# Sidharthshanu/Gossip-protocol-with-power-law

Hardware: AMD Instinct MI355X
Metric: gossip edge-deliveries/s (GTEPS) & HBM roofline %, 2^24 nodes x 4096 msgs (higher is better)
Workload: dtype u64

## Files before the change

### gossip-protocol-with-power-law_amd/csrc/driver.hip

```cpp
#include <hip/hip_runtime.h>

#include <cstdlib>
#include <rccl/rccl.h>

#include <algorithm>
#include <cmath>
#include <cstring>
#include <string>
#include <vector>

#include "gp_device.h"
#include "xplan.h"

namespace gp {

static thread_local std::string g_err;
int set_error(int code, const std::string& msg) {
  g_err = msg;
  return code;
}
int copy_sync(Ctx* c, void* dst, const void* src, size_t bytes, hipMemcpyKind kind) {
  if (bytes == 0) return 0;
  GP_HIP(hipMemcpyAsync(dst, src, bytes, kind, c->stream));
  GP_HIP(hipStreamSynchronize(c->stream));
// ... 268 lines not shown
  a.lm_next = c->lm_write_now ? c->d_lmw[c->cur ^ 1] : nullptr;
  a.cmk = c->cml_read_now ? c->d_cmk[c->cur] : nullptr;
  a.cml = c->cml_read_now ? c->d_cml[c->cur] : nullptr;
  a.cmk_next = c->cml_write_now ? c->d_cmk[c->cur ^ 1] : nullptr;
  a.cml_next = c->cml_write_now ? c->d_cml[c->cur ^ 1] : nullptr;
  a.frx = c->d_frx[0] ? c->d_frx[c->cur] : nullptr;
  a.frx_next = c->d_frx[0] ? c->d_frx[c->cur ^ 1] : nullptr;
  a.frx_rows = c->frx_rows;
  a.done_at = c->d_done_at;
  a.gcol = c->d_gcol;
  a.midx = c->d_midx;
  a.cmask = c->d_cmask;
  a.early_exit = c->early_exit_now ? 1 : 0;
  a.dprobe = c->dprobe_now ? 1 : 0;
  a.alias = c->alias_now ? 1 : 0;
  a.ulist = c->ulist_read_now ? c->d_ulist[c->ul_cur] : nullptr;
  a.ulist_n = c->ulist_read_now ? c->ulist_n : 0;
  a.ulist_next = c->ulist_emit_now ? c->d_ulist[c->ul_cur ^ 1] : nullptr;
  a.fpop_next = c->d_fpop[c->cur ^ 1];
  a.seenpop = c->d_seenpop;
  a.first = c->cfg.track_first ? c->d_first : nullptr;
  a.digest = c->cfg.track_digest ? c->d_digest : nullptr;
  a.state = c->d_state;
  a.deg_live = c->d_deg_live;
  a.partial = c->d_stats + 64;
  a.hub_items = c->d_hub_items;
  a.hubs = c->d_hubs;
  a.hub_item_ptr = c->d_hub_item_ptr;
  a.hub_partial = c->d_hub_partial;
  a.hub_pnz = c->d_hub_pnz;
  a.hub_done = c->d_hub_done;
  if (++c->hub_epoch == 0) c->hub_epoch = 1;
  a.hub_epoch = c->hub_epoch;
  a.vbegin = 0;
  a.nloc = c->nloc();
  a.m_total = c->m;
  a.wbase = c->cfg.msg_word_base;
  a.rr = c->round + 1;
  a.hub_thr = c->cfg.hub_threshold;
  a.orp = c->directed ? c->d_out_row_ptr : c->d_row_ptr;
  a.ocol = c->directed ? c->d_out_col : c->d_col;
  a.acc = c->d_acc;
  a.tbits = c->d_tbits;
  a.touched = c->d_touched;
  a.active = c->d_active;
  a.big = c->d_big;
  a.stats = c->d_stats;
}


#ifndef GP_EE_DIV
#define GP_EE_DIV 16.0
#endif
#ifndef GP_EE_DIV_NARROW
#define GP_EE_DIV_NARROW 64.0
#endif
static int launch_expand(Ctx* c) {
  if (alive_on(c))
    GP_HIP(hipMemsetAsync(c->d_alive + (size_t)(c->cur ^ 1) * c->words, 0, (size_t)c->words * 8, c->stream));
  const int r = c->round;
  const double ee_div = c->words <= 8 ? GP_EE_DIV_NARROW : GP_EE_DIV;
  c->early_exit_now = c->cfg.early_exit != 0 &&
                      ((double)c->prev_new_bits * ee_div >= (double)c->n * (double)c->m ||
                       (double)c->held_bits * 2.0 >= (double)c->n * (double)c->m);
  const u64 inj = (size_t)r < c->inj_arcs.size() ? (u64)c->inj_arcs[(size_t)r] : 0ull;
  const double est = (double)((r == 0 ? 0ull : c->prev_next_arcs) + inj);
// ... 626 lines not shown
```

### gossip-protocol-with-power-law_amd/csrc/gp_device.h

```cpp
#pragma once
#include <hip/hip_runtime.h>

#include <algorithm>
#include <cstdint>

#include "gp_internal.h"

namespace gp {

typedef unsigned long long u64;
typedef u64 u64x2 __attribute__((ext_vector_type(2)));

constexpr int BLOCK = 256;
constexpr int WAVES = BLOCK / 64;
constexpr int GS = 256 / BLOCK;
#ifndef GP_EXPAND_BLOCK
#define GP_EXPAND_BLOCK 64
#endif
constexpr int EBLOCK = GP_EXPAND_BLOCK;
constexpr int EWAVES = EBLOCK / 64;
constexpr int HBLOCK = 256;
constexpr int HWAVES = HBLOCK / 64;
constexpr int NPART = 2048;

// ... 115 lines not shown
  const uint32_t* __restrict__ done_at;
  uint32_t* __restrict__ fpop_next;
  u64* __restrict__ frx;
  u64* __restrict__ frx_next;
  int64_t frx_rows;
  uint32_t* __restrict__ seenpop;
  uint8_t* __restrict__ first;
  u64* __restrict__ digest;
  uint8_t* __restrict__ state;
  const int32_t* __restrict__ deg_live;
  u64* __restrict__ partial;
  const HubItem* __restrict__ hub_items;
  const int32_t* __restrict__ hubs;
  const int32_t* __restrict__ hub_item_ptr;
  u64* __restrict__ hub_partial;
  uint32_t* __restrict__ hub_pnz;
  uint32_t* __restrict__ hub_done;
  uint32_t hub_epoch;
  const int64_t* __restrict__ orp;
  const int32_t* __restrict__ ocol;
  u64* __restrict__ acc;
  u64* __restrict__ tbits;
  const u64* __restrict__ nbits;
  int32_t* __restrict__ touched;
  const int32_t* __restrict__ active;
  const int32_t* __restrict__ big;
  u64* __restrict__ stats;
  int64_t vbegin, nloc;
  int64_t n_items;
  int32_t m_total;
  int32_t wbase;
  int32_t rr;
  int32_t hub_thr;
};

constexpr uint8_t SLOT_NONE = 0xFF;
constexpr uint8_t SLOT_PARKED = 2;
constexpr uint8_t SLOT_CMASK = 3;
constexpr uint8_t LMN_ALIAS = 0x10;

constexpr int CML_WORDS = 16;
constexpr int CML_MAXW = CML_WORDS - 1;

#ifndef GP_DETECT_BLOCKS_PER_CU
#define GP_DETECT_BLOCKS_PER_CU 16
#endif
constexpr double SUMMARY_RATIO = 256.0;
#define EXPAND_BOUNDS __launch_bounds__(EBLOCK)
#ifndef GP_ROWS_IN_FLIGHT
#define GP_ROWS_IN_FLIGHT 4
#endif
#ifndef GP_ROWS_IN_FLIGHT_64
#define GP_ROWS_IN_FLIGHT_64 3
#endif
#ifndef GP_ROWS_IN_FLIGHT_NARROW
#define GP_ROWS_IN_FLIGHT_NARROW 2
#endif
template <int W>
struct RowsInFlight {
  static constexpr int value = W >= 64 ? GP_ROWS_IN_FLIGHT_64 : W == 8 ? GP_ROWS_IN_FLIGHT_NARROW : GP_ROWS_IN_FLIGHT;
};

constexpr int PRE_IDS = 8;
constexpr int PRE_MAX_DEG = 16;
#ifndef GP_WAVE_PRE_MAX
#define GP_WAVE_PRE_MAX 64
// ... 519 lines not shown
    const uint32_t hi = (uint32_t)__shfl_xor((int)nib, 1);
    if (!(lane & 1) && li < a.nloc) a.lm_next[li >> 1] = (uint8_t)(nib | (hi << 4));
  }
  if constexpr (LDS::kCml) {
    if (a.cmk_next) {
      const u64 dm = __ballot(!need || L.tot[lane] == 0u || L.cd[lane] != 0);
      if (lane == 0 && li < a.nloc) a.cmk_next[li >> 6] = dm;
    }
  }
}



inline int grid_for(int64_t work, int64_t per_block) {
  int64_t g = (work + per_block - 1) / per_block;
  if (g < 1) g = 1;
  if (g > (int64_t)0x7fffffff) g = 0x7fffffff;
  return (int)g;
}
inline bool alive_on(const Ctx* c) { return c->d_alive != nullptr && c->liveness_active; }
inline bool alive_now(const Ctx* c) { return alive_on(c) && c->alive_from >= 0 && c->round >= c->alive_from; }
inline bool state_ready(const Ctx* c) { return c->d_sp != nullptr && c->d_slot[0] != nullptr; }

int launch_round_kernels(Ctx* c, const ExpandArgs& a);
template <int W> void launch_expand_flat_w(Ctx* c, const ExpandArgs& a);
void launch_expand_rec(Ctx* c, const ExpandArgs& a);
void launch_mklm(Ctx* c, const ExpandArgs& a);
void launch_arcmask(Ctx* c);
template <int W> void launch_fixup_rows_w(Ctx* c);
template <int W> void launch_park_w(Ctx* c);
template <int W> void launch_push_w(Ctx* c, ExpandArgs a);
template <int W> void launch_split_push_w(Ctx* c, const ExpandArgs& a);
template <int W> void launch_acc_clear_w(Ctx* c);
template <int W> void launch_hubs_w(Ctx* c, const ExpandArgs& a, bool unfiltered, bool lines);
int launch_liveness(Ctx* c);
constexpr int DET_CAP = 16384;

}
```

### gossip-protocol-with-power-law_amd/csrc/gp_internal.h

```cpp
#pragma once
#include <hip/hip_runtime.h>
#include <rccl/rccl.h>

#include <cstdint>
#include <map>
#include <string>
#include <vector>

#include "../../include/gossip_capi.h"
#include "gp_common.h"

namespace gp {

typedef unsigned long long u64;

enum StatSlot {
  S_INJECTED = 0, S_LOST, S_NEW_BITS, S_RECEIVERS, S_SENDS, S_ACTIVE, S_CRASHED,
  S_REPORTS, S_REMOVALS, S_DUP, S_ARCS, S_GATHERED, S_SEEN_READ, S_WRITTEN,
  S_VISITED, S_NEXT_ARCS, S_ATOMICS, S_ROW_BYTES,
  S_XROWS, S_XBYTES,
  S_DNB,
  S_LM_ROWS,
  S_ALIASED,
  NST,
  S_XERR = NST + 1,
  S_REPORT_CURSOR = 26, S_CAND, S_ACTIVE_CURSOR, S_BIG_CURSOR, S_TOUCH_CURSOR, S_DET_BIG,
  S_ULIST
};
static_assert(S_XERR < S_REPORT_CURSOR, "S_XERR must be inside the all-reduced counter slots");

struct HubItem {
  int32_t v;
  int32_t hub;
  int64_t beg, end;
};

struct InjectSpan { int64_t off; int64_t cnt; };

struct Ctx {
  int device = 0;
  hipStream_t stream = nullptr;
  hipEvent_t ev[6] = {};
  gp_config cfg{};

  int64_t n = 0, nnz = 0;
  int directed = 0;
  int64_t* d_row_ptr = nullptr;
  int32_t* d_col = nullptr;
  int64_t* d_out_row_ptr = nullptr;
  int32_t* d_out_col = nullptr;
  int32_t* d_deg_out = nullptr;
  int32_t* d_comp = nullptr;
  std::vector<int64_t> h_row_ptr;

  int32_t rank = 0, nranks = 1;
  std::vector<int64_t> h_bounds;
  int64_t vbegin = 0, vend = 0;
  int64_t n_alloc = 0;
  bool local = false;
  int64_t nghost = 0, nextra = 0;
  int64_t nnz_l = 0;
  int32_t* d_l2g = nullptr;
  std::vector<int32_t> h_l2g;
  std::vector<int32_t> h_comp_g;
  std::vector<int32_t> h_deg_g;
  int64_t base_nv = 0;
  std::vector<int64_t> h_bnd_ptr;
  std::vector<int64_t> h_gh_ptr;
  int64_t n_bnd = 0, n_bvx = 0;
  int32_t* d_bnd_e = nullptr;
  int32_t* d_bnd_k = nullptr;
  int32_t* d_bvx_v = nullptr;
  int32_t* d_bvx_ptr = nullptr;
  int32_t* d_bvx_t = nullptr;
  int64_t* d_bnd_ptr = nullptr;
// ... 102 lines not shown
  uint32_t* d_done_at0 = nullptr;
  u64* d_cmask0 = nullptr;
  uint32_t* d_lostcnt = nullptr;
  int32_t cmask_rows = 0;
  bool done_dirty = false;
  u64* d_msg_cov = nullptr;
  u64* d_msg_fwd = nullptr;
  u64* d_alive = nullptr;
  u64* d_bc_keys = nullptr;
  uint32_t* d_bc_part = nullptr;
  size_t bc_part_words = 0;
  int64_t bc_split = 0;
  u64* d_fin_comp = nullptr;
  u64* d_fin_list = nullptr;
  int32_t fin_comp_rows = 0;
  gp_report* d_reports = nullptr;
  int64_t report_cap = 0;
  u64* d_stats = nullptr;
  u64* h_stats = nullptr;
  int32_t round = 0;
  bool liveness_active = false;
  int32_t alive_from = -1;
  bool pending_crash = false;
  bool msg_forwards_valid = true;
  int64_t last_reports = 0;

  std::vector<HubItem> h_hub_items;
  HubItem* d_hub_items = nullptr;
  int32_t* d_hubs = nullptr;
  int32_t* d_hub_item_ptr = nullptr;
  u64* d_hub_partial = nullptr;
  uint32_t* d_hub_pnz = nullptr;
  int64_t n_hubs = 0, n_hub_items = 0;

  ncclComm_t comm = nullptr;

  ncclComm_t jcomm = nullptr;
  gp_allgather_fn jhost = nullptr;
  void* jhost_user = nullptr;
  int32_t jrank = 0, jnranks = 0;
  u64* d_hist = nullptr;
  int32_t hist_cap = 0, hist_rounds = 0;
  int64_t hist_nw = 0;
  bool hist_valid = true;
  std::vector<gp_round_stats> run_stats;
  int32_t fin_round = -1;
  u64* d_jscr = nullptr;
  size_t jscr_words = 0;
  u64* d_jdig = nullptr;
  size_t jdig_words = 0;
  u64* d_jcf = nullptr;
  int32_t jm = 0;
  bool j_ready = false, j_fwd_valid = false, j_dig_valid = false;

  int cu_count = 256;

  int64_t nloc() const { return vend - vbegin; }
  int64_t to_local(int64_t g) const;

};

int set_error(int code, const std::string& msg);
#define GP_HIP(call)                                                              \
  do {                                                                            \
    hipError_t _e = (call);                                                       \
    if (_e != hipSuccess)                                                         \
// ... 56 lines not shown
```

### gossip-protocol-with-power-law_amd/csrc/hub.hip

```cpp
#include "gp_device.h"

namespace gp {

template <int W, int MODE>
__global__ __launch_bounds__(HBLOCK) void k_hub_partial(ExpandArgs a) {
  constexpr int LPR = Geo<W>::LPR;
  __shared__ WaveLds s_w[HWAVES];
  const int lane = threadIdx.x & 63;
  const int wib = uniform(threadIdx.x >> 6);
  const int g = lane / LPR, lw = lane % LPR;
  WaveStats st;
  ws_zero(st);
  const int64_t it = (int64_t)blockIdx.x * HWAVES + wib;
  if (it < a.n_items) {
    const HubItem h = a.hub_items[it];
    const int64_t i = h.v - a.vbegin;
    u64x2 acc = {0, 0};
    if (!(a.state[h.v] & (ST_DOWN | ST_SATED)) && a.seenpop[i] < a.done_at[h.v]) {
      const bool ee = a.early_exit != 0;
      u64x2 want = {0, 0};
      if (ee) want = early_exit_target<W>(a, h.v, s_w[wib], g, lw, a.sp[h.v], a.midx[h.v]);
      const int64_t hend = a.prehi ? min(h.end, a.row_ptr[h.v] + (int64_t)a.prehi[h.v]) : h.end;
      constexpr int64_t SUB = 512;
      for (int64_t s0 = h.beg; s0 < hend; s0 += SUB) {
        if (ee && a.hub_done) {
          uint32_t f = 0;
          if (lane == 0) f = __hip_atomic_load(a.hub_done + h.hub, __ATOMIC_RELAXED, __HIP_MEMORY_SCOPE_AGENT);
          if ((uint32_t)__builtin_amdgcn_readfirstlane((int)f) == a.hub_epoch) break;
        }
        gather_scan<W, MODE, W == 64 && (MODE == SCAN_FILTERED || MODE == SCAN_UNFILTERED)>(
            a, s0, min(hend, s0 + SUB), s_w[wib], lane, g, lw, acc, st, ee, want);
        if (ee) {
          u64x2 t = acc;
          reduce_slots<W>(t);
          const u64x2 miss = want & ~t;
          if (!__any((miss.x | miss.y) != 0ull)) {
            if (lane == 0 && a.hub_done)
              __hip_atomic_store(a.hub_done + h.hub, a.hub_epoch, __ATOMIC_RELAXED, __HIP_MEMORY_SCOPE_AGENT);
            break;
          }
        }
      }
      reduce_slots<W>(acc);
    }
    const bool nz = __any((acc.x | acc.y) != 0);
    if (nz && g == 0) store_piece<W>(a.hub_partial, it, lw, acc);
    if (lane == 0) a.hub_pnz[it] = nz ? 1u : 0u;
  }
  flush_stats(st, a.partial);
}

template <int W>
__global__ __launch_bounds__(HBLOCK) void k_hub_final(ExpandArgs a) {
  constexpr int LPR = Geo<W>::LPR;
  __shared__ WaveLds s_w[HWAVES];
  const int lane = threadIdx.x & 63;
  const int wib = uniform(threadIdx.x >> 6);
  const int g = lane / LPR, lw = lane % LPR;
  WaveStats st;
  ws_zero(st);
  const int64_t h = (int64_t)blockIdx.x * HWAVES + wib;
  alive_zero<W>(a, s_w[wib].alive, lane);
  wave_sync_lds();
  if (h < a.n_items) {
    const int v = a.hubs[h];
    const int64_t i = v - a.vbegin;
    if ((a.state[v] & (ST_DOWN | ST_SATED)) || a.seenpop[i] >= a.done_at[v]) {
      if (lane == 0) a.fpop_next[v] = 0;
    } else {
      st.add(S_VISITED, 1);
      u64x2 acc = {0, 0};
      const int p0 = a.hub_item_ptr[h], p1 = a.hub_item_ptr[h + 1];
      if (g == 0) {
        for (int p = p0; p < p1; ++p)
          if (a.hub_pnz[p]) acc |= load_piece<W>(a.hub_partial, p, lw);
        if (a.prehi) acc |= load_piece<W>(a.acc, v, lw);
      }
      if (a.sate && a.early_exit && a.alive) {
        u64x2 rem = {0, 0};
        if (g == 0) {
          const u64x2 sv = load_seen<W>(a, v, a.sp[v], lw);
          rem = load_piece<W>(a.cmask, a.midx[v], lw) & load_piece<W>(a.alive, 0, lw) & ~sv & ~acc;
        }
        if (!__any((rem.x | rem.y) != 0ull) && lane == 0) a.state[v] |= ST_SATED;
      }
      finish_row<W>(a, v, i, acc, lane, g, lw, st, s_w[wib], false, a.sp[v]);
    }
  }
  alive_flush<W>(a, s_w[wib].alive, lane);
  flush_stats(st, a.partial);
}


template <int W>
void launch_hubs_w(Ctx* c, const ExpandArgs& a, bool unfiltered, bool lines) {
  ExpandArgs h = a;
  h.n_items = c->n_hub_items;
  const dim3 grid(grid_for(h.n_items, HWAVES));
  bool done = false;
  if constexpr (W == 64) {
    if (lines && !unfiltered) {
      hipLaunchKernelGGL((k_hub_partial<W, SCAN_FILTERED | SCAN_LINES>), grid, dim3(HBLOCK), 0, c->stream, h);
      done = true;
    }
  }
  if (done) {
  } else if (unfiltered)
    hipLaunchKernelGGL((k_hub_partial<W, SCAN_UNFILTERED>), grid, dim3(HBLOCK), 0, c->stream, h);
  else
    hipLaunchKernelGGL((k_hub_partial<W, SCAN_FILTERED>), grid, dim3(HBLOCK), 0, c->stream, h);
  h.n_items = c->n_hubs;
  hipLaunchKernelGGL(k_hub_final<W>, dim3(grid_for(h.n_items, HWAVES)), dim3(HBLOCK), 0, c->stream, h);
}
template void launch_hubs_w<1>(Ctx*, const ExpandArgs&, bool, bool);
template void launch_hubs_w<2>(Ctx*, const ExpandArgs&, bool, bool);
template void launch_hubs_w<4>(Ctx*, const ExpandArgs&, bool, bool);
template void launch_hubs_w<8>(Ctx*, const ExpandArgs&, bool, bool);
template void launch_hubs_w<16>(Ctx*, const ExpandArgs&, bool, bool);
template void launch_hubs_w<32>(Ctx*, const ExpandArgs&, bool, bool);
template void launch_hubs_w<64>(Ctx*, const ExpandArgs&, bool, bool);

}
```

### gossip-protocol-with-power-law_amd/csrc/pull.hip

```cpp
#include "pull_groups.h"

namespace gp {

template <int W, int MODE>
__global__ EXPAND_BOUNDS __attribute__((amdgpu_waves_per_eu(1))) void k_expand(ExpandArgs a) {
  constexpr int LPR = Geo<W>::LPR;
  __shared__ LDS_OF(MODE) s_w[EWAVES];
  const int lane = threadIdx.x & 63;
  const int wib = uniform(threadIdx.x >> 6);
  const int g = lane / LPR, lw = lane % LPR;
  auto& L = s_w[wib];
  constexpr bool ALIVE = (MODE & SCAN_ALIVE) != 0;
  constexpr bool DPROBE = (MODE & SCAN_DPROBE) != 0;
  constexpr bool LIST = (MODE & SCAN_LIST) != 0;
  constexpr bool QUADS = (MODE & SCAN_QUADS) != 0;
  constexpr int SCAN = MODE & ~(SCAN_ALIVE | SCAN_DPROBE | SCAN_LIST | SCAN_QUADS);
  constexpr bool EMIT = W == 64 && (SCAN == SCAN_FILTERED || SCAN == SCAN_UNFILTERED);
  constexpr bool ALIASABLE = W == 64 && !ALIVE && (SCAN == SCAN_FILTERED || SCAN == SCAN_UNFILTERED);
  constexpr bool GPAIRS = W == 64 && QUADS && !ALIVE && SCAN == SCAN_UNFILTERED && !LIST;
  constexpr bool GGROUPS = (W == 32 || W == 16) && QUADS && !ALIVE && SCAN == SCAN_UNFILTERED && !LIST;
  WaveStats st;
  ws_zero<EWAVES>(st);
  const int64_t base = ((int64_t)blockIdx.x * EWAVES + wib) * 64;
  if (base < (LIST ? a.ulist_n : a.nloc)) {
    const int64_t li = base + lane;
    const bool valid = LIST ? li < a.ulist_n : li < a.nloc;
    const int64_t vi = LIST ? (valid ? (int64_t)a.ulist[li] : 0) : li;
    bool need = false, act = false, dnb = false;
    u64 tw = 0;
    if constexpr ((MODE & 3) == SCAN_PRE) {
      if (a.prehi) tw = a.tbits[base >> 6];
    }
    u64 sends = 0;
    uint32_t slot_of = SLOT_NONE;
    uint32_t pre_arcs = 0;
    bool small = false;
    if (valid) {
      const int v = (int)(a.vbegin + vi);
      if constexpr (!LIST) {
        const uint32_t fp = a.fpop[v];
        act = fp != 0u;
        if (act) sends = (u64)fp * (u64)(uint32_t)max(a.deg_live[v], 0);
      }
      const int64_t b = a.row_ptr[v], e = a.row_ptr[v + 1];
      L.rp[lane] = b;
      if constexpr (LIST) {
        L.re[lane] = e;
        L.vid[lane] = v;
      } else {
        if (lane == 63 || li + 1 == a.nloc) L.rp[lane + 1] = e;
      }
      const bool hub = e - b > a.hub_thr;
      need = !(a.state[v] & (ST_DOWN | ST_SATED)) && a.seenpop[vi] < a.done_at[v] && !hub && e > b;
      if constexpr (GPAIRS) small = e - b <= 32;
      if constexpr (GGROUPS) small = e - b <= Geo<W>::LPR;
      if constexpr ((MODE & 3) == SCAN_MASKED) need = need && mask_any(a.amask, b, e);
// ... 323 lines not shown
    p.mode = scan;
  } else if (a.ulist && built(scan | SCAN_LIST)) {
    p.kernel = PULL_LIST;
    p.mode = scan | SCAN_LIST | (alive_ee ? SCAN_ALIVE : a.dprobe ? SCAN_DPROBE : 0);
  } else if (a.nloc > 0 && unf) {
    p.kernel = PULL_RECEIVER;
    const bool half_held = (double)c->held_bits * 2.0 >= (double)c->n * (double)c->m;
    if (alive_ee && built(scan | SCAN_ALIVE))
      p.mode = scan | SCAN_ALIVE | (half_held && built(scan | SCAN_ALIVE | SCAN_QUADS) ? SCAN_QUADS : 0);
    else if (a.dprobe && built(scan | SCAN_DPROBE)) p.mode = scan | SCAN_DPROBE;
    else if ((a.alias || a.near_done) && built(scan | SCAN_QUADS)) p.mode = scan | SCAN_QUADS;
    else p.mode = scan;
  } else if (a.nloc > 0) {
    p.kernel = PULL_RECEIVER;
    const int pre = c->prefilter_now ? SCAN_PRE : SCAN_FILTERED;
    if (a.dprobe && built(scan | SCAN_DPROBE)) {
      p.mode = scan | SCAN_DPROBE;
    } else if (p.masked) {
      p.mode = SCAN_MASKED;
    } else if ((a.cmk || a.cmk_next) && built(pre | SCAN_CML)) {
      if (a.cmk && !a.early_exit && !c->prefilter_now && !a.alive) p.kernel = PULL_RECORD;
      else p.mode = pre | SCAN_CML;
    } else if (alive_ee && built(pre | SCAN_ALIVE)) {
      p.mode = pre | SCAN_ALIVE;
    } else if (p.lines) {
      p.mode = SCAN_FILTERED | SCAN_LINES;
    } else {
      p.mode = pre;
    }
  }
  return p;
}

template <int W>
static bool launch_expand_w(Ctx* c, ExpandArgs a) {
  if (c->mode_push) {
    launch_push_w<W>(c, a);
    return true;
  }
  if (a.unfiltered && c->liveness_active) launch_park_w<W>(c);
  if (a.unfiltered) launch_fixup_rows_w<W>(c);
  const PullChoice p = choose_pull(c, a, W);
  if (p.masked) launch_arcmask(c);
  (void)hipEventRecord(c->ev[4], c->stream);
  if (a.prehi) launch_split_push_w<W>(c, a);
  if (p.lines && !p.lm_from_commits) launch_mklm(c, a);
  bool ok = true;
  switch (p.kernel) {
    case PULL_FLAT:
      if constexpr (W <= 32) launch_expand_flat_w<W>(c, a);
      else ok = false;
      break;
    case PULL_LIST: ok = launch_k_expand<W>(c, a, a.ulist_n, p.mode); break;
    case PULL_RECEIVER: ok = launch_k_expand<W>(c, a, a.nloc, p.mode); break;
    case PULL_RECORD: launch_expand_rec(c, a); break;
    case PULL_NONE: break;
  }
  if (p.mode & SCAN_LINES) {
    c->lines_ran = true;
    c->lines_from_commits = p.lm_from_commits;
  }
  if (c->n_hub_items > 0) launch_hubs_w<W>(c, a, a.unfiltered != 0, c->lines_ran);
  if (a.prehi) launch_acc_clear_w<W>(c);
  (void)hipEventRecord(c->ev[5], c->stream);
  return ok;
}

int launch_round_kernels(Ctx* c, const ExpandArgs& a) {
  bool ok = false;
  switch (c->words) {
    case 1: ok = launch_expand_w<1>(c, a); break;
    case 2: ok = launch_expand_w<2>(c, a); break;
    case 4: ok = launch_expand_w<4>(c, a); break;
    case 8: ok = launch_expand_w<8>(c, a); break;
    case 16: ok = launch_expand_w<16>(c, a); break;
    case 32: ok = launch_expand_w<32>(c, a); break;
    case 64: ok = launch_expand_w<64>(c, a); break;
    default: return set_error(GP_EINVAL, "unsupported word count");
  }
  GP_HIP(hipGetLastError());
  if (!ok) return set_error(GP_EINVAL, "the round chose a pull kernel that is not built for this row width");
  return 0;
}

}
```

### gossip-protocol-with-power-law_amd/csrc/setup.hip

```cpp
#include <cstdlib>
#include <cstring>
#include <string>
#include <vector>

#include "gp_device.h"
#include "xplan.h"

namespace gp {

__device__ __forceinline__ int32_t cc_parent(const int32_t* p, int32_t x) {
  return __hip_atomic_load(p + x, __ATOMIC_RELAXED, __HIP_MEMORY_SCOPE_AGENT);
}
__device__ int32_t cc_find(int32_t* __restrict__ parent, int32_t x) {
  int32_t p = cc_parent(parent, x);
  while (p != x) {
    const int32_t g = cc_parent(parent, p);
    if (g != p) __hip_atomic_store(parent + x, g, __ATOMIC_RELAXED, __HIP_MEMORY_SCOPE_AGENT);
    x = p;
    p = g;
  }
  return x;
}
__global__ void k_cc_init(int32_t* __restrict__ parent, int64_t n) {
  const int64_t v = (int64_t)blockIdx.x * blockDim.x + threadIdx.x;
  if (v < n) parent[v] = (int32_t)v;
}
constexpr int CC_SAMPLE = 2;
__device__ void cc_link(int32_t* __restrict__ parent, int32_t a, int32_t b) {
  while (true) {
    a = cc_find(parent, a);
    b = cc_find(parent, b);
    if (a == b) return;
    if (a < b) {
      const int32_t t = a;
      a = b;
      b = t;
    }
// ... 38 lines not shown
                                int64_t groups, const int32_t* __restrict__ comp, uint32_t* __restrict__ cnt) {
  const int64_t k = (int64_t)blockIdx.x * blockDim.x + threadIdx.x;
  if (k < groups) atomicAdd(cnt + comp[origin[k]], gcnt[k]);
}
__global__ void k_done_at(const int32_t* __restrict__ comp, const uint32_t* __restrict__ cnt,
                          uint32_t* __restrict__ done_at, int64_t n) {
  const int64_t v = (int64_t)blockIdx.x * blockDim.x + threadIdx.x;
  if (v < n) done_at[v] = cnt[comp[v]];
}
__global__ void k_degree(const int64_t* __restrict__ rp, int32_t* __restrict__ deg, int64_t n) {
  const int64_t v = (int64_t)blockIdx.x * blockDim.x + threadIdx.x;
  if (v < n) deg[v] = (int32_t)(rp[v + 1] - rp[v]);
}

__global__ __launch_bounds__(BLOCK) void k_nbsum(const int64_t* __restrict__ rp, const int32_t* __restrict__ col,
                                                 const u64* __restrict__ val, const int32_t* __restrict__ vtx,
                                                 int64_t cnt, u64* __restrict__ out) {
  const int lane = threadIdx.x & 63;
  const int64_t nw = (int64_t)gridDim.x * (BLOCK / 64);
  for (int64_t k = (int64_t)blockIdx.x * (BLOCK / 64) + (threadIdx.x >> 6); k < cnt; k += nw) {
    const int64_t v = vtx ? vtx[k] : k;
    const int64_t b = rp[v], e = rp[v + 1];
    u64 s = 0;
    for (int64_t j = b + lane; j < e; j += 64) {
      const int32_t u = col[j];
      s += val ? val[u] : (u64)(rp[u + 1] - rp[u]);
    }
#pragma unroll
    for (int off = 32; off > 0; off >>= 1) s += __shfl_xor(s, off);
    if (lane == 0) out[k] = s;
  }
}


int build_hubs(Ctx* c) {
  c->h_hub_items.clear();
  std::vector<int32_t> hubs, ptr;
  const int64_t thr = c->cfg.hub_threshold;
  if (!c->h_row_ptr.empty()) {
    for (int64_t v = 0; v < c->nloc(); ++v) {
      const int64_t b = c->h_row_ptr[v], e = c->h_row_ptr[v + 1];
      if (e - b <= thr) continue;
      ptr.push_back((int32_t)c->h_hub_items.size());
      for (int64_t j = b; j < e; j += thr)
        c->h_hub_items.push_back(HubItem{(int32_t)v, (int32_t)hubs.size(), j, std::min(e, j + thr)});
      hubs.push_back((int32_t)v);
    }
  }
  ptr.push_back((int32_t)c->h_hub_items.size());
  c->n_hubs = (int64_t)hubs.size();
  c->n_hub_items = (int64_t)c->h_hub_items.size();
  GP_TRY(dalloc(&c->d_hub_items, c->h_hub_items.size()));
  GP_TRY(dalloc(&c->d_hubs, hubs.size()));
  GP_TRY(dalloc(&c->d_hub_item_ptr, ptr.size()));
  GP_TRY(dalloc(&c->d_hub_pnz, c->h_hub_items.size()));
  GP_TRY(dalloc(&c->d_hub_done, std::max<size_t>(hubs.size(), 1)));
  GP_HIP(hipMemsetAsync(c->d_hub_done, 0, std::max<size_t>(hubs.size(), 1) * 4, c->stream));
  c->hub_epoch = 0;
  if (!c->h_hub_items.empty())
    GP_TRY(copy_sync(c, c->d_hub_items, c->h_hub_items.data(), c->h_hub_items.size() * sizeof(HubItem),
                     hipMemcpyHostToDevice));
  if (!hubs.empty())
    GP_TRY(copy_sync(c, c->d_hubs, hubs.data(), hubs.size() * sizeof(int32_t), hipMemcpyHostToDevice));
  GP_TRY(copy_sync(c, c->d_hub_item_ptr, ptr.data(), ptr.size() * sizeof(int32_t), hipMemcpyHostToDevice));
  if (c->words > 0) GP_TRY(dalloc(&c->d_hub_partial, c->h_hub_items.size() * (size_t)c->words));
  return 0;
}

static void free_state(Ctx* c);

static int set_partition(Ctx* c, int32_t rank, int32_t nranks) {
  if (nranks < 1 || rank < 0 || rank >= nranks) return set_error(GP_EINVAL, "bad rank/nranks");
  if (c->local && (rank != c->rank || nranks != c->nranks))
    return set_error(GP_ESTATE, "a partitioned context keeps its partition: reload the overlay to change it");
  if (c->local) return 0;
  if (nranks > 1 && c->directed)
    return set_error(GP_EINVAL, "vertex partitions need an undirected overlay (ghost rows are in-neighbours)");
  c->rank = rank;
  c->nranks = nranks;
  c->h_bounds = partition_bounds(c->n, nranks, c->cfg.partition_by_arcs,
                                 c->h_row_ptr.size() == (size_t)c->n + 1 ? c->h_row_ptr.data() : nullptr);
  c->vbegin = c->h_bounds[(size_t)rank];
  c->vend = c->h_bounds[(size_t)rank + 1];
  c->n_alloc = c->n;
  c->base_nv = c->n;
  if (nranks > 1) {
    free_state(c);
    GP_TRY(localize(c));
  }
  return build_hubs(c);
}

static void free_rows(Ctx* c) {
  dfree(&c->d_rows);
  c->d_slot[0] = c->d_slot[1] = c->d_acc = nullptr;
}

static void free_state(Ctx* c) {
  dfree(&c->d_slot[2]);
// ... 243 lines not shown
  cfg->prefilter_pct = 20;
  cfg->compact_rows = 0;
  cfg->unfiltered_pct = 90;
  cfg->msg_word_base = 0;
  cfg->flat_max_words = 16;
  cfg->summary_min_n = 1ll << 25;
  cfg->partition_by_arcs = 0;
#ifndef GP_SPLIT_DEG_DEFAULT
#define GP_SPLIT_DEG_DEFAULT 128
#endif
#ifndef GP_SPLIT_MAX_PERMILLE
#define GP_SPLIT_MAX_PERMILLE 10
#endif
  cfg->split_deg = GP_SPLIT_DEG_DEFAULT;
  cfg->split_max_permille = GP_SPLIT_MAX_PERMILLE;
}

int gp_create(int device, gp_ctx** out) {
  if (!out) return set_error(GP_EINVAL, "null out");
  *out = nullptr;
  int ndev = 0;
  GP_HIP(hipGetDeviceCount(&ndev));
  if (device < 0 || device >= ndev) return set_error(GP_EINVAL, "device index out of range");
  GP_HIP(hipSetDevice(device));
  gp_ctx* c = new gp_ctx();
  c->device = device;
  gp_default_config(&c->cfg);
  hipDeviceProp_t prop;
  if (hipGetDeviceProperties(&prop, device) == hipSuccess) c->cu_count = prop.multiProcessorCount;
  if (hipStreamCreateWithFlags(&c->stream, hipStreamNonBlocking) != hipSuccess) {
    delete c;
    return set_error(GP_EHIP, "hipStreamCreate failed");
  }
  for (auto& e : c->ev) (void)hipEventCreate(&e);
  if (dalloc(&c->d_stats, 64 + (size_t)NPART * NST) != 0) {
    gp_destroy(c);
    return GP_ENOMEM;
  }
  (void)hipMemsetAsync(c->d_stats, 0, (64 + (size_t)NPART * NST) * sizeof(u64), c->stream);
  (void)hipStreamSynchronize(c->stream);
  (void)hipHostMalloc((void**)&c->h_stats, 64 * sizeof(u64), hipHostMallocDefault);
  *out = c;
  return 0;
}

void gp_destroy(gp_ctx* c) {
  if (!c) return;
  (void)hipSetDevice(c->device);
  if (c->stream) (void)hipStreamSynchronize(c->stream);
  if (c->comm) (void)ncclCommDestroy(c->comm);
  shard_free(c);
  dfree(&c->d_row_ptr); dfree(&c->d_col); dfree(&c->d_out_row_ptr); dfree(&c->d_out_col);
  dfree(&c->d_deg_out); dfree(&c->d_comp); dfree(&c->d_abits); dfree(&c->d_dbits); dfree(&c->d_lm); dfree(&c->d_lmw[0]); dfree(&c->d_lmw[1]); dfree(&c->d_sbits); dfree(&c->d_amask); dfree(&c->d_cml[0]); dfree(&c->d_cml[1]); dfree(&c->d_cmk[0]); dfree(&c->d_cmk[1]); dfree(&c->d_done_at);
  dfree(&c->d_done_at0); dfree(&c->d_cmask0); dfree(&c->d_lostcnt); dfree(&c->d_alive);
  dfree(&c->d_gcol); dfree(&c->d_prehi); dfree(&c->d_midx); dfree(&c->d_cmask);
  dfree(&c->d_tbits); dfree(&c->d_nbits); dfree(&c->d_touched); dfree(&c->d_active); dfree(&c->d_big);
  dfree(&c->d_inj_origin); dfree(&c->d_inj_bits); dfree(&c->d_inj_cnt);
  dfree(&c->d_slot[2]);
  free_rows(c);
  for (int k = 0; k < 2; ++k) { dfree(&c->d_frx[k]); dfree(&c->d_fpop[k]); }
  dfree(&c->d_sp); dfree(&c->d_ws);
  dfree(&c->d_ulist[0]); dfree(&c->d_ulist[1]);
  dfree(&c->d_seenpop); dfree(&c->d_first); dfree(&c->d_digest);
  dfree(&c->d_state); dfree(&c->d_miss); dfree(&c->d_deg_live); dfree(&c->d_cand);
  dfree(&c->d_det_big); dfree(&c->d_det_pre); dfree(&c->d_det_live); dfree(&c->d_det_cur); dfree(&c->d_det_base);
  dfree(&c->d_msg_cov); dfree(&c->d_reports); dfree(&c->d_stats);
  dfree(&c->d_hub_items); dfree(&c->d_hubs); dfree(&c->d_hub_item_ptr);
  dfree(&c->d_hub_partial); dfree(&c->d_hub_pnz); dfree(&c->d_hub_done);
  bitcount_free(c);
  if (c->h_stats) (void)hipHostFree(c->h_stats);
  for (auto& e : c->ev) if (e) (void)hipEventDestroy(e);
  if (c->stream) (void)hipStreamDestroy(c->stream);
  delete c;
}

int gp_configure(gp_ctx* c, const gp_config* cfg) {
  if (!c || !cfg) return set_error(GP_EINVAL, "null argument");
  if (cfg->p_fail < 0.0 || !(cfg->p_fail <= 1.0)) return set_error(GP_EINVAL, "p_fail must be in [0,1]");
  if (cfg->miss_threshold < 1 || cfg->miss_threshold > 254) return set_error(GP_EINVAL, "miss_threshold in [1,254]");
  if (cfg->hub_threshold < 64) return set_error(GP_EINVAL, "hub_threshold must be >= 64");
  if (cfg->report_capacity < 0) return set_error(GP_EINVAL, "report_capacity < 0");
  if (cfg->msg_word_base < 0) return set_error(GP_EINVAL, "msg_word_base < 0");
  if (cfg->prefilter_pct < 0) return set_error(GP_EINVAL, "prefilter_pct < 0");
  if (cfg->summary_min_n < 0) return set_error(GP_EINVAL, "summary_min_n < 0");
  if (cfg->compact_rows != 0 && cfg->compact_rows != 1) return set_error(GP_EINVAL, "compact_rows must be 0 or 1");
  if (cfg->arc_mask_permille < 0) return set_error(GP_EINVAL, "arc_mask_permille < 0");
  if (cfg->partition_by_arcs != 0 && cfg->partition_by_arcs != 1)
    return set_error(GP_EINVAL, "partition_by_arcs must be 0 or 1");
  if (cfg->split_deg < 0) return set_error(GP_EINVAL, "split_deg must be >= 0");
  if (cfg->split_max_permille < 0) return set_error(GP_EINVAL, "split_max_permille must be >= 0");
  if (c->local && cfg->partition_by_arcs != c->cfg.partition_by_arcs)
    return set_error(GP_ESTATE, "a partitioned context keeps its partition: reload the overlay to change it");
  GP_HIP(hipSetDevice(c->device));
  const bool hub_changed = cfg->hub_threshold != c->cfg.hub_threshold;
  c->cfg = *cfg;
  if (c->n > 0 && hub_changed) GP_TRY(build_hubs(c));
  if (state_ready(c)) GP_TRY(alloc_state(c));
  return 0;
}

int gp_load_graph(gp_ctx* c, int64_t n, int64_t nnz, const int64_t* row_ptr, const int32_t* col,
                  int32_t directed, const int64_t* out_row_ptr, const int32_t* out_col) {
  if (!c || !row_ptr || (nnz > 0 && !col)) return set_error(GP_EINVAL, "null argument");
  if (n <= 0 || n >= (int64_t)0x7fffffff) return set_error(GP_EINVAL, "n out of range");
// ... 282 lines not shown
```

Measured before the change: 25940.

## Overlap hub partial kernel on side stream and schedule heavy row blocks first

Splits hub processing into a partial kernel launched on a new side stream, forked and joined with events so it can run concurrently with the main pull kernel, and a final kernel kept on the main stream. Shrinks the hub-partial block to one wave. Adds a host-built block order that puts 64-row blocks with long non-hub rows first, sorted by their longest row, and the pull kernel remaps block indices through it to cut tail imbalance. The cost is an extra stream and events, an indirection load per wave, and host setup work, plus possible contention between concurrent kernels.

```diff
diff --git a/gossip-protocol-with-power-law_amd/csrc/block_order.h b/gossip-protocol-with-power-law_amd/csrc/block_order.h
--- /dev/null
+++ b/gossip-protocol-with-power-law_amd/csrc/block_order.h
@@ -0,0 +1,36 @@
+#pragma once
+#include <algorithm>
+#include <cstdint>
+#include <utility>
+#include <vector>
+
+namespace gp {
+
+inline std::vector<int32_t> block_order(const int64_t* row_ptr, int64_t nloc, int64_t hub_thr, int64_t cut) {
+  const int64_t nb = (nloc + 63) / 64;
+  std::vector<int32_t> order;
+  order.reserve((size_t)nb);
+  std::vector<std::pair<int64_t, int32_t>> heavy;
+  std::vector<uint8_t> first((size_t)nb, 0);
+  for (int64_t b = 0; b < nb; ++b) {
+    int64_t longest = 0;
+    const int64_t v1 = std::min(nloc, (b + 1) * 64);
+    for (int64_t v = b * 64; v < v1; ++v) {
+      const int64_t d = row_ptr[v + 1] - row_ptr[v];
+      if (d <= hub_thr) longest = std::max(longest, d);
+    }
+    if (longest > cut) {
+      heavy.emplace_back(longest, (int32_t)b);
+      first[(size_t)b] = 1;
+    }
+  }
+  std::sort(heavy.begin(), heavy.end(), [](const std::pair<int64_t, int32_t>& x, const std::pair<int64_t, int32_t>& y) {
+    return x.first != y.first ? x.first > y.first : x.second < y.second;
+  });
+  for (const auto& h : heavy) order.push_back(h.second);
+  for (int64_t b = 0; b < nb; ++b)
+    if (!first[(size_t)b]) order.push_back((int32_t)b);
+  return order;
+}
+
+}
diff --git a/gossip-protocol-with-power-law_amd/csrc/driver.hip b/gossip-protocol-with-power-law_amd/csrc/driver.hip
--- a/gossip-protocol-with-power-law_amd/csrc/driver.hip
+++ b/gossip-protocol-with-power-law_amd/csrc/driver.hip
@@ -324,6 +324,7 @@
   a.hub_done = c->d_hub_done;
   if (++c->hub_epoch == 0) c->hub_epoch = 1;
   a.hub_epoch = c->hub_epoch;
+  a.border = c->d_border;
   a.vbegin = 0;
   a.nloc = c->nloc();
   a.m_total = c->m;
diff --git a/gossip-protocol-with-power-law_amd/csrc/gp_device.h b/gossip-protocol-with-power-law_amd/csrc/gp_device.h
--- a/gossip-protocol-with-power-law_amd/csrc/gp_device.h
+++ b/gossip-protocol-with-power-law_amd/csrc/gp_device.h
@@ -171,6 +171,7 @@
   int32_t wbase;
   int32_t rr;
   int32_t hub_thr;
+  const int32_t* __restrict__ border;
 };
 
 constexpr uint8_t SLOT_NONE = 0xFF;
@@ -756,7 +757,8 @@
 template <int W> void launch_push_w(Ctx* c, ExpandArgs a);
 template <int W> void launch_split_push_w(Ctx* c, const ExpandArgs& a);
 template <int W> void launch_acc_clear_w(Ctx* c);
-template <int W> void launch_hubs_w(Ctx* c, const ExpandArgs& a, bool unfiltered, bool lines);
+template <int W> void launch_hub_partial_w(Ctx* c, const ExpandArgs& a, bool unfiltered, bool lines, hipStream_t s);
+template <int W> void launch_hub_final_w(Ctx* c, const ExpandArgs& a);
 int launch_liveness(Ctx* c);
 constexpr int DET_CAP = 16384;
 
diff --git a/gossip-protocol-with-power-law_amd/csrc/gp_internal.h b/gossip-protocol-with-power-law_amd/csrc/gp_internal.h
--- a/gossip-protocol-with-power-law_amd/csrc/gp_internal.h
+++ b/gossip-protocol-with-power-law_amd/csrc/gp_internal.h
@@ -41,6 +41,8 @@
   int device = 0;
   hipStream_t stream = nullptr;
   hipEvent_t ev[6] = {};
+  hipStream_t side = nullptr;
+  hipEvent_t ev_fork = nullptr, ev_join = nullptr;
   gp_config cfg{};
 
   int64_t n = 0, nnz = 0;
@@ -209,6 +211,7 @@
   u64* d_hub_partial = nullptr;
   uint32_t* d_hub_pnz = nullptr;
   int64_t n_hubs = 0, n_hub_items = 0;
+  int32_t* d_border = nullptr;
 
   ncclComm_t comm = nullptr;
 
diff --git a/gossip-protocol-with-power-law_amd/csrc/hub.hip b/gossip-protocol-with-power-law_amd/csrc/hub.hip
--- a/gossip-protocol-with-power-law_amd/csrc/hub.hip
+++ b/gossip-protocol-with-power-law_amd/csrc/hub.hip
@@ -2,16 +2,19 @@
 
 namespace gp {
 
+constexpr int HPBLOCK = 64;
+constexpr int HPWAVES = HPBLOCK / 64;
+
 template <int W, int MODE>
-__global__ __launch_bounds__(HBLOCK) void k_hub_partial(ExpandArgs a) {
+__global__ __launch_bounds__(HPBLOCK) void k_hub_partial(ExpandArgs a) {
   constexpr int LPR = Geo<W>::LPR;
-  __shared__ WaveLds s_w[HWAVES];
+  __shared__ WaveLds s_w[HPWAVES];
   const int lane = threadIdx.x & 63;
   const int wib = uniform(threadIdx.x >> 6);
   const int g = lane / LPR, lw = lane % LPR;
   WaveStats st;
-  ws_zero(st);
-  const int64_t it = (int64_t)blockIdx.x * HWAVES + wib;
+  ws_zero<HPWAVES>(st);
+  const int64_t it = (int64_t)blockIdx.x * HPWAVES + wib;
   if (it < a.n_items) {
     const HubItem h = a.hub_items[it];
     const int64_t i = h.v - a.vbegin;
@@ -47,7 +50,7 @@
     if (nz && g == 0) store_piece<W>(a.hub_partial, it, lw, acc);
     if (lane == 0) a.hub_pnz[it] = nz ? 1u : 0u;
   }
-  flush_stats(st, a.partial);
+  flush_stats<HPWAVES>(st, a.partial);
 }
 
 template <int W>
@@ -93,31 +96,33 @@
 
 
 template <int W>
-void launch_hubs_w(Ctx* c, const ExpandArgs& a, bool unfiltered, bool lines) {
+void launch_hub_partial_w(Ctx* c, const ExpandArgs& a, bool unfiltered, bool lines, hipStream_t s) {
   ExpandArgs h = a;
   h.n_items = c->n_hub_items;
-  const dim3 grid(grid_for(h.n_items, HWAVES));
+  const dim3 grid(grid_for(h.n_items, HPWAVES));
   bool done = false;
   if constexpr (W == 64) {
     if (lines && !unfiltered) {
-      hipLaunchKernelGGL((k_hub_partial<W, SCAN_FILTERED | SCAN_LINES>), grid, dim3(HBLOCK), 0, c->stream, h);
+      hipLaunchKernelGGL((k_hub_partial<W, SCAN_FILTERED | SCAN_LINES>), grid, dim3(HPBLOCK), 0, s, h);
       done = true;
     }
   }
   if (done) {
   } else if (unfiltered)
-    hipLaunchKernelGGL((k_hub_partial<W, SCAN_UNFILTERED>), grid, dim3(HBLOCK), 0, c->stream, h);
+    hipLaunchKernelGGL((k_hub_partial<W, SCAN_UNFILTERED>), grid, dim3(HPBLOCK), 0, s, h);
   else
-    hipLaunchKernelGGL((k_hub_partial<W, SCAN_FILTERED>), grid, dim3(HBLOCK), 0, c->stream, h);
+    hipLaunchKernelGGL((k_hub_partial<W, SCAN_FILTERED>), grid, dim3(HPBLOCK), 0, s, h);
+}
+template <int W>
+void launch_hub_final_w(Ctx* c, const ExpandArgs& a) {
+  ExpandArgs h = a;
   h.n_items = c->n_hubs;
   hipLaunchKernelGGL(k_hub_final<W>, dim3(grid_for(h.n_items, HWAVES)), dim3(HBLOCK), 0, c->stream, h);
 }
-template void launch_hubs_w<1>(Ctx*, const ExpandArgs&, bool, bool);
-template void launch_hubs_w<2>(Ctx*, const ExpandArgs&, bool, bool);
-template void launch_hubs_w<4>(Ctx*, const ExpandArgs&, bool, bool);
-template void launch_hubs_w<8>(Ctx*, const ExpandArgs&, bool, bool);
-template void launch_hubs_w<16>(Ctx*, const ExpandArgs&, bool, bool);
-template void launch_hubs_w<32>(Ctx*, const ExpandArgs&, bool, bool);
-template void launch_hubs_w<64>(Ctx*, const ExpandArgs&, bool, bool);
+#define V(W)                                                                                   \
+  template void launch_hub_partial_w<W>(Ctx*, const ExpandArgs&, bool, bool, hipStream_t);     \
+  template void launch_hub_final_w<W>(Ctx*, const ExpandArgs&);
+V(1) V(2) V(4) V(8) V(16) V(32) V(64)
+#undef V
 
 }
diff --git a/gossip-protocol-with-power-law_amd/csrc/pull.hip b/gossip-protocol-with-power-law_amd/csrc/pull.hip
--- a/gossip-protocol-with-power-law_amd/csrc/pull.hip
+++ b/gossip-protocol-with-power-law_amd/csrc/pull.hip
@@ -21,7 +21,11 @@
   constexpr bool GGROUPS = (W == 32 || W == 16) && QUADS && !ALIVE && SCAN == SCAN_UNFILTERED && !LIST;
   WaveStats st;
   ws_zero<EWAVES>(st);
-  const int64_t base = ((int64_t)blockIdx.x * EWAVES + wib) * 64;
+  int64_t blk = (int64_t)blockIdx.x * EWAVES + wib;
+  if constexpr (!LIST) {
+    if (a.border && blk * 64 < a.nloc) blk = uniform(a.border[blk]);
+  }
+  const int64_t base = blk * 64;
   if (base < (LIST ? a.ulist_n : a.nloc)) {
     const int64_t li = base + lane;
     const bool valid = LIST ? li < a.ulist_n : li < a.nloc;
@@ -411,11 +415,12 @@
   return p;
 }
 
+enum { PULL_OK = 0, PULL_NOT_BUILT = 1, PULL_ORDER_FAILED = 2 };
 template <int W>
-static bool launch_expand_w(Ctx* c, ExpandArgs a) {
+static int launch_expand_w(Ctx* c, ExpandArgs a) {
   if (c->mode_push) {
     launch_push_w<W>(c, a);
-    return true;
+    return PULL_OK;
   }
   if (a.unfiltered && c->liveness_active) launch_park_w<W>(c);
   if (a.unfiltered) launch_fixup_rows_w<W>(c);
@@ -424,41 +429,55 @@
   (void)hipEventRecord(c->ev[4], c->stream);
   if (a.prehi) launch_split_push_w<W>(c, a);
   if (p.lines && !p.lm_from_commits) launch_mklm(c, a);
-  bool ok = true;
+  if (p.mode & SCAN_LINES) {
+    c->lines_ran = true;
+    c->lines_from_commits = p.lm_from_commits;
+  }
+  const bool hubs = c->n_hub_items > 0;
+  bool order_ok = true;
+  if (hubs) {
+    order_ok = hipEventRecord(c->ev_fork, c->stream) == hipSuccess &&
+               hipStreamWaitEvent(c->side, c->ev_fork, 0) == hipSuccess;
+    if (order_ok) {
+      launch_hub_partial_w<W>(c, a, a.unfiltered != 0, c->lines_ran, c->side);
+      order_ok = hipEventRecord(c->ev_join, c->side) == hipSuccess;
+    }
+  }
+  int rc = PULL_OK;
   switch (p.kernel) {
     case PULL_FLAT:
       if constexpr (W <= 32) launch_expand_flat_w<W>(c, a);
-      else ok = false;
+      else rc = PULL_NOT_BUILT;
       break;
-    case PULL_LIST: ok = launch_k_expand<W>(c, a, a.ulist_n, p.mode); break;
-    case PULL_RECEIVER: ok = launch_k_expand<W>(c, a, a.nloc, p.mode); break;
+    case PULL_LIST: if (!launch_k_expand<W>(c, a, a.ulist_n, p.mode)) rc = PULL_NOT_BUILT; break;
+    case PULL_RECEIVER: if (!launch_k_expand<W>(c, a, a.nloc, p.mode)) rc = PULL_NOT_BUILT; break;
     case PULL_RECORD: launch_expand_rec(c, a); break;
     case PULL_NONE: break;
   }
-  if (p.mode & SCAN_LINES) {
-    c->lines_ran = true;
-    c->lines_from_commits = p.lm_from_commits;
-  }
-  if (c->n_hub_items > 0) launch_hubs_w<W>(c, a, a.unfiltered != 0, c->lines_ran);
+  if (hubs) {
+    order_ok = order_ok && hipStreamWaitEvent(c->stream, c->ev_join, 0) == hipSuccess;
+    if (order_ok) launch_hub_final_w<W>(c, a);
+  }
   if (a.prehi) launch_acc_clear_w<W>(c);
   (void)hipEventRecord(c->ev[5], c->stream);
-  return ok;
+  return order_ok ? rc : PULL_ORDER_FAILED;
 }
 
 int launch_round_kernels(Ctx* c, const ExpandArgs& a) {
-  bool ok = false;
+  int rc = PULL_OK;
   switch (c->words) {
-    case 1: ok = launch_expand_w<1>(c, a); break;
-    case 2: ok = launch_expand_w<2>(c, a); break;
-    case 4: ok = launch_expand_w<4>(c, a); break;
-    case 8: ok = launch_expand_w<8>(c, a); break;
-    case 16: ok = launch_expand_w<16>(c, a); break;
-    case 32: ok = launch_expand_w<32>(c, a); break;
-    case 64: ok = launch_expand_w<64>(c, a); break;
+    case 1: rc = launch_expand_w<1>(c, a); break;
+    case 2: rc = launch_expand_w<2>(c, a); break;
+    case 4: rc = launch_expand_w<4>(c, a); break;
+    case 8: rc = launch_expand_w<8>(c, a); break;
+    case 16: rc = launch_expand_w<16>(c, a); break;
+    case 32: rc = launch_expand_w<32>(c, a); break;
+    case 64: rc = launch_expand_w<64>(c, a); break;
     default: return set_error(GP_EINVAL, "unsupported word count");
   }
   GP_HIP(hipGetLastError());
-  if (!ok) return set_error(GP_EINVAL, "the round chose a pull kernel that is not built for this row width");
+  if (rc == PULL_ORDER_FAILED) return set_error(GP_EHIP, "the hub chunks could not be ordered against the round's pull kernel");
+  if (rc == PULL_NOT_BUILT) return set_error(GP_EINVAL, "the round chose a pull kernel that is not built for this row width");
   return 0;
 }
 
diff --git a/gossip-protocol-with-power-law_amd/csrc/setup.hip b/gossip-protocol-with-power-law_amd/csrc/setup.hip
--- a/gossip-protocol-with-power-law_amd/csrc/setup.hip
+++ b/gossip-protocol-with-power-law_amd/csrc/setup.hip
@@ -3,6 +3,7 @@
 #include <string>
 #include <vector>
 
+#include "block_order.h"
 #include "gp_device.h"
 #include "xplan.h"
 
@@ -107,6 +108,17 @@
   }
 }
 
+
+#ifndef GP_BLOCK_ORDER_CUT
+#define GP_BLOCK_ORDER_CUT 1024
+#endif
+static int build_block_order(Ctx* c) {
+  dfree(&c->d_border);
+  if (c->h_row_ptr.empty() || c->nloc() <= 0) return 0;
+  const std::vector<int32_t> order = block_order(c->h_row_ptr.data(), c->nloc(), c->cfg.hub_threshold, GP_BLOCK_ORDER_CUT);
+  GP_TRY(dalloc(&c->d_border, order.size()));
+  return copy_sync(c, c->d_border, order.data(), order.size() * sizeof(int32_t), hipMemcpyHostToDevice);
+}
 
 int build_hubs(Ctx* c) {
   c->h_hub_items.clear();
@@ -139,7 +151,7 @@
     GP_TRY(copy_sync(c, c->d_hubs, hubs.data(), hubs.size() * sizeof(int32_t), hipMemcpyHostToDevice));
   GP_TRY(copy_sync(c, c->d_hub_item_ptr, ptr.data(), ptr.size() * sizeof(int32_t), hipMemcpyHostToDevice));
   if (c->words > 0) GP_TRY(dalloc(&c->d_hub_partial, c->h_hub_items.size() * (size_t)c->words));
-  return 0;
+  return build_block_order(c);
 }
 
 static void free_state(Ctx* c);
@@ -449,7 +461,16 @@
     delete c;
     return set_error(GP_EHIP, "hipStreamCreate failed");
   }
+  if (hipStreamCreateWithFlags(&c->side, hipStreamNonBlocking) != hipSuccess) {
+    gp_destroy(c);
+    return set_error(GP_EHIP, "hipStreamCreate failed");
+  }
   for (auto& e : c->ev) (void)hipEventCreate(&e);
+  if (hipEventCreateWithFlags(&c->ev_fork, hipEventDisableTiming) != hipSuccess ||
+      hipEventCreateWithFlags(&c->ev_join, hipEventDisableTiming) != hipSuccess) {
+    gp_destroy(c);
+    return set_error(GP_EHIP, "hipEventCreate failed");
+  }
   if (dalloc(&c->d_stats, 64 + (size_t)NPART * NST) != 0) {
     gp_destroy(c);
     return GP_ENOMEM;
@@ -465,6 +486,7 @@
   if (!c) return;
   (void)hipSetDevice(c->device);
   if (c->stream) (void)hipStreamSynchronize(c->stream);
+  if (c->side) (void)hipStreamSynchronize(c->side);
   if (c->comm) (void)ncclCommDestroy(c->comm);
   shard_free(c);
   dfree(&c->d_row_ptr); dfree(&c->d_col); dfree(&c->d_out_row_ptr); dfree(&c->d_out_col);
@@ -483,10 +505,13 @@
   dfree(&c->d_det_big); dfree(&c->d_det_pre); dfree(&c->d_det_live); dfree(&c->d_det_cur); dfree(&c->d_det_base);
   dfree(&c->d_msg_cov); dfree(&c->d_reports); dfree(&c->d_stats);
   dfree(&c->d_hub_items); dfree(&c->d_hubs); dfree(&c->d_hub_item_ptr);
-  dfree(&c->d_hub_partial); dfree(&c->d_hub_pnz); dfree(&c->d_hub_done);
+  dfree(&c->d_hub_partial); dfree(&c->d_hub_pnz); dfree(&c->d_hub_done); dfree(&c->d_border);
   bitcount_free(c);
   if (c->h_stats) (void)hipHostFree(c->h_stats);
   for (auto& e : c->ev) if (e) (void)hipEventDestroy(e);
+  if (c->ev_fork) (void)hipEventDestroy(c->ev_fork);
+  if (c->ev_join) (void)hipEventDestroy(c->ev_join);
+  if (c->side) (void)hipStreamDestroy(c->side);
   if (c->stream) (void)hipStreamDestroy(c->stream);
   delete c;
 }
```

Result: faster. 27000 (median of 6 runs) (+4.1%).
